# 0xPARC/plonkathon

Measured on NVIDIA H100. Metric: plonk_proofs_per_s_2^20_gates, higher is better.
Workload: dtype u256 (BN254 Fr/Fq integers, 8x32-bit Montgomery limbs)

## Files before the change

### plonkathon_b200/csrc/curve.cuh

```cuda
#pragma once
#include "field.cuh"

namespace pb200 {

struct alignas(16) G1Affine {
  Fq x, y;
};

struct alignas(16) G1XYZZ {
  Fq X, Y, ZZ, ZZZ;
  PB_HD bool is_inf() const { return ZZ.is_zero(); }
  static PB_HD G1XYZZ identity() {
    G1XYZZ r;
    r.X = Fq::zero(); r.Y = Fq::zero(); r.ZZ = Fq::zero(); r.ZZZ = Fq::zero();
    return r;
  }
};

PB_HD G1XYZZ g1_from_affine(const G1Affine& p) {
  G1XYZZ r;
  r.X = p.x; r.Y = p.y; r.ZZ = Fq::one(); r.ZZZ = Fq::one();
  return r;
}

PB_HD void g1_double_affine(G1XYZZ& acc, const G1Affine& p) {
  Fq U = fp_dbl(p.y);
  Fq V = fp_sqr(U);
  Fq W = fp_mul(U, V);
  Fq S = fp_mul(p.x, V);
  Fq M = fp_sqr(p.x);
  M = fp_add(fp_dbl(M), M);
  Fq X3 = fp_sub(fp_sqr(M), fp_dbl(S));
  acc.Y = fp_sub(fp_mul(M, fp_sub(S, X3)), fp_mul(W, p.y));
  acc.X = X3;
  acc.ZZ = V;
  acc.ZZZ = W;
}

PB_HD void g1_double(G1XYZZ& a) {
  if (a.is_inf()) return;
  Fq U = fp_dbl(a.Y);
  Fq V = fp_sqr(U);
  Fq W = fp_mul(U, V);
  Fq S = fp_mul(a.X, V);
  Fq M = fp_sqr(a.X);
  M = fp_add(fp_dbl(M), M);
  Fq X3 = fp_sub(fp_sqr(M), fp_dbl(S));
  a.Y = fp_sub(fp_mul(M, fp_sub(S, X3)), fp_mul(W, a.Y));
  a.X = X3;
  a.ZZ = fp_mul(V, a.ZZ);
  a.ZZZ = fp_mul(W, a.ZZZ);
}

PB_HD void g1_add_mixed(G1XYZZ& acc, const G1Affine& p) {
  if (acc.is_inf()) {
    acc = g1_from_affine(p);
    return;
  }
  Fq U2 = fp_mul(p.x, acc.ZZ);
  Fq S2 = fp_mul(p.y, acc.ZZZ);
  Fq Pd = fp_sub(U2, acc.X);
  Fq Rd = fp_sub(S2, acc.Y);
  if (Pd.is_zero()) {
    if (Rd.is_zero()) g1_double_affine(acc, p);
    else acc = G1XYZZ::identity();
    return;
  }
  Fq PP = fp_sqr(Pd);
  Fq PPP = fp_mul(Pd, PP);
  Fq Q = fp_mul(acc.X, PP);
  Fq X3 = fp_sub(fp_sub(fp_sqr(Rd), PPP), fp_dbl(Q));
  acc.Y = fp_sub(fp_mul(Rd, fp_sub(Q, X3)), fp_mul(acc.Y, PPP));
  acc.X = X3;
  acc.ZZ = fp_mul(acc.ZZ, PP);
  acc.ZZZ = fp_mul(acc.ZZZ, PPP);
}

PB_HD void g1_add_mixed_uniform(G1XYZZ& acc, const G1Affine& p) {
  const bool was_inf = acc.is_inf();
  Fq U2 = fp_mul(p.x, acc.ZZ);
  Fq S2 = fp_mul(p.y, acc.ZZZ);
  Fq Pd = fp_sub(U2, acc.X);
  Fq Rd = fp_sub(S2, acc.Y);
  if (!was_inf && Pd.is_zero()) {
    if (Rd.is_zero()) g1_double_affine(acc, p);
    else acc = G1XYZZ::identity();
    return;
  }
  Fq PP = fp_sqr(Pd);
  Fq PPP = fp_mul(Pd, PP);
  Fq Q = fp_mul(acc.X, PP);
  Fq X3 = fp_sub(fp_sub(fp_sqr(Rd), PPP), fp_dbl(Q));
  Fq Y3 = fp_sub(fp_mul(Rd, fp_sub(Q, X3)), fp_mul(acc.Y, PPP));
  Fq ZZ3 = fp_mul(acc.ZZ, PP);
  Fq ZZZ3 = fp_mul(acc.ZZZ, PPP);
  const Fq one = Fq::one();
#pragma unroll
  for (int i = 0; i < 8; i++) {
    acc.X.v[i] = was_inf ? p.x.v[i] : X3.v[i];
    acc.Y.v[i] = was_inf ? p.y.v[i] : Y3.v[i];
    acc.ZZ.v[i] = was_inf ? one.v[i] : ZZ3.v[i];
    acc.ZZZ.v[i] = was_inf ? one.v[i] : ZZZ3.v[i];
  }
}

PB_HD void g1_add(G1XYZZ& acc, const G1XYZZ& q) {
  if (q.is_inf()) return;
  if (acc.is_inf()) {
    acc = q;
    return;
  }
  Fq U1 = fp_mul(acc.X, q.ZZ);
  Fq U2 = fp_mul(q.X, acc.ZZ);
  Fq S1 = fp_mul(acc.Y, q.ZZZ);
  Fq S2 = fp_mul(q.Y, acc.ZZZ);
  Fq Pd = fp_sub(U2, U1);
  Fq Rd = fp_sub(S2, S1);
  if (Pd.is_zero()) {
    if (Rd.is_zero()) g1_double(acc);
    else acc = G1XYZZ::identity();
    return;
  }
  Fq PP = fp_sqr(Pd);
  Fq PPP = fp_mul(Pd, PP);
  Fq Q = fp_mul(U1, PP);
  Fq X3 = fp_sub(fp_sub(fp_sqr(Rd), PPP), fp_dbl(Q));
  acc.Y = fp_sub(fp_mul(Rd, fp_sub(Q, X3)), fp_mul(S1, PPP));
  acc.X = X3;
  acc.ZZ = fp_mul(fp_mul(acc.ZZ, q.ZZ), PP);
  acc.ZZZ = fp_mul(fp_mul(acc.ZZZ, q.ZZZ), PPP);
}

PB_HD void g1_add_uniform(G1XYZZ& acc, const G1XYZZ& q) {
  const bool a_inf = acc.is_inf(), q_inf = q.is_inf();
  Fq U1 = fp_mul(acc.X, q.ZZ);
  Fq U2 = fp_mul(q.X, acc.ZZ);
  Fq S1 = fp_mul(acc.Y, q.ZZZ);
  Fq S2 = fp_mul(q.Y, acc.ZZZ);
  Fq Pd = fp_sub(U2, U1);
  Fq Rd = fp_sub(S2, S1);
  if (!a_inf && !q_inf && Pd.is_zero()) {
    if (Rd.is_zero()) g1_double(acc);
    else acc = G1XYZZ::identity();
    return;
  }
  Fq PP = fp_sqr(Pd);
  Fq PPP = fp_mul(Pd, PP);
  Fq Q = fp_mul(U1, PP);
  Fq X3 = fp_sub(fp_sub(fp_sqr(Rd), PPP), fp_dbl(Q));
  Fq Y3 = fp_sub(fp_mul(Rd, fp_sub(Q, X3)), fp_mul(S1, PPP));
  Fq ZZ3 = fp_mul(fp_mul(acc.ZZ, q.ZZ), PP);
  Fq ZZZ3 = fp_mul(fp_mul(acc.ZZZ, q.ZZZ), PPP);
#pragma unroll
  for (int i = 0; i < 8; i++) {
    acc.X.v[i] = q_inf ? acc.X.v[i] : (a_inf ? q.X.v[i] : X3.v[i]);
    acc.Y.v[i] = q_inf ? acc.Y.v[i] : (a_inf ? q.Y.v[i] : Y3.v[i]);
    acc.ZZ.v[i] = q_inf ? acc.ZZ.v[i] : (a_inf ? q.ZZ.v[i] : ZZ3.v[i]);
    acc.ZZZ.v[i] = q_inf ? acc.ZZZ.v[i] : (a_inf ? q.ZZZ.v[i] : ZZZ3.v[i]);
  }
}

PB_HD G1Affine g1_neg_affine(const G1Affine& p) {
  G1Affine r;
  r.x = p.x;
  r.y = fp_neg(p.y);
  return r;
}

PB_HD bool g1_to_affine(const G1XYZZ& a, G1Affine& out) {
  if (a.is_inf()) {
    out.x = Fq::zero();
    out.y = Fq::zero();
    return true;
  }
  Fq A = fp_inv(a.ZZZ);
  Fq izz = fp_sqr(fp_mul(a.ZZ, A));
  out.x = fp_mul(a.X, izz);
  out.y = fp_mul(a.Y, A);
  return false;
}

}
```

### plonkathon_b200/csrc/field.cuh

```cuda
#pragma once
#include <stdint.h>

#if defined(__CUDACC__)
#define PB_HD __host__ __device__ __forceinline__
#define PB_D __device__ __forceinline__
#else
#define PB_HD inline
#define PB_D inline
#endif

namespace pb200 {

#if defined(__CUDA_ARCH__)
PB_D uint32_t add_cc(uint32_t a, uint32_t b) { uint32_t r; asm volatile("add.cc.u32 %0, %1, %2;" : "=r"(r) : "r"(a), "r"(b)); return r; }
PB_D uint32_t addc_cc(uint32_t a, uint32_t b) { uint32_t r; asm volatile("addc.cc.u32 %0, %1, %2;" : "=r"(r) : "r"(a), "r"(b)); return r; }
PB_D uint32_t addc(uint32_t a, uint32_t b) { uint32_t r; asm volatile("addc.u32 %0, %1, %2;" : "=r"(r) : "r"(a), "r"(b)); return r; }
PB_D uint32_t sub_cc(uint32_t a, uint32_t b) { uint32_t r; asm volatile("sub.cc.u32 %0, %1, %2;" : "=r"(r) : "r"(a), "r"(b)); return r; }
PB_D uint32_t subc_cc(uint32_t a, uint32_t b) { uint32_t r; asm volatile("subc.cc.u32 %0, %1, %2;" : "=r"(r) : "r"(a), "r"(b)); return r; }
PB_D uint32_t subc(uint32_t a, uint32_t b) { uint32_t r; asm volatile("subc.u32 %0, %1, %2;" : "=r"(r) : "r"(a), "r"(b)); return r; }
PB_D uint32_t mul_lo(uint32_t a, uint32_t b) { uint32_t r; asm volatile("mul.lo.u32 %0, %1, %2;" : "=r"(r) : "r"(a), "r"(b)); return r; }
PB_D uint32_t mul_hi(uint32_t a, uint32_t b) { uint32_t r; asm volatile("mul.hi.u32 %0, %1, %2;" : "=r"(r) : "r"(a), "r"(b)); return r; }
PB_D uint32_t mad_lo_cc(uint32_t a, uint32_t b, uint32_t c) { uint32_t r; asm volatile("mad.lo.cc.u32 %0, %1, %2, %3;" : "=r"(r) : "r"(a), "r"(b), "r"(c)); return r; }
PB_D uint32_t madc_lo_cc(uint32_t a, uint32_t b, uint32_t c) { uint32_t r; asm volatile("madc.lo.cc.u32 %0, %1, %2, %3;" : "=r"(r) : "r"(a), "r"(b), "r"(c)); return r; }
PB_D uint32_t madc_hi_cc(uint32_t a, uint32_t b, uint32_t c) { uint32_t r; asm volatile("madc.hi.cc.u32 %0, %1, %2, %3;" : "=r"(r) : "r"(a), "r"(b), "r"(c)); return r; }
// ... 143 lines not shown
      U[j] = madc_lo_cc(a[j], b, U[j]);
      U[j + 1] = madc_hi_cc(a[j], b, U[j + 1]);
    }
    uint32_t c1 = addc(0u, 0u);
    w = V[1];
    V[0] = mad_lo_cc(a[1], b, V[2]);
    V[1] = madc_hi_cc(a[1], b, V[3]);
    V[2] = madc_lo_cc(a[3], b, V[4]);
    V[3] = madc_hi_cc(a[3], b, V[5]);
    V[4] = madc_lo_cc(a[5], b, V[6]);
    V[5] = madc_hi_cc(a[5], b, V[7]);
    V[6] = madc_lo_cc(a[7], b, 0u);
    V[7] = madc_hi(a[7], b, c1);
  }
  uint32_t m = mul_lo(U[0] + w, P::NP0);
  fp_mad_row_mod<P, 1>(V, m);
  fp_mad_row_mod<P, 0>(U, m);
  V[7] = addc(V[7], 0u);
}

#if !defined(__CUDA_ARCH__) && defined(PB_HOST_FAST_MUL)
template <class P>
inline Fp<P> fp_mul_host64(const Fp<P>& a, const Fp<P>& b) {
  typedef unsigned __int128 u128;
  uint64_t A[4], B[4], M[4], T[6] = {0, 0, 0, 0, 0, 0};
  for (int i = 0; i < 4; i++) {
    A[i] = (uint64_t)a.v[2 * i] | ((uint64_t)a.v[2 * i + 1] << 32);
    B[i] = (uint64_t)b.v[2 * i] | ((uint64_t)b.v[2 * i + 1] << 32);
    M[i] = (uint64_t)P::p(2 * i) | ((uint64_t)P::p(2 * i + 1) << 32);
  }
  uint64_t np = 1;
  for (int k = 0; k < 6; k++) np *= 2 - M[0] * np;
  np = (uint64_t)0 - np;
  for (int i = 0; i < 4; i++) {
    u128 c = 0;
    for (int j = 0; j < 4; j++) { c += (u128)A[j] * B[i] + T[j]; T[j] = (uint64_t)c; c >>= 64; }
    c += T[4]; T[4] = (uint64_t)c; T[5] = (uint64_t)(c >> 64);
    uint64_t m = T[0] * np;
    c = (u128)m * M[0] + T[0]; c >>= 64;
    for (int j = 1; j < 4; j++) { c += (u128)m * M[j] + T[j]; T[j - 1] = (uint64_t)c; c >>= 64; }
    c += T[4]; T[3] = (uint64_t)c; T[4] = T[5] + (uint64_t)(c >> 64); T[5] = 0;
  }
  uint64_t r[4]; u128 br = 0; bool ge = T[4] != 0;
  if (!ge) { ge = true; for (int i = 3; i >= 0; i--) { if (T[i] != M[i]) { ge = T[i] > M[i]; break; } } }
  if (ge) { for (int i = 0; i < 4; i++) { u128 d = (u128)T[i] - M[i] - (uint64_t)br; r[i] = (uint64_t)d; br = (d >> 64) & 1; } }
  else { for (int i = 0; i < 4; i++) r[i] = T[i]; }
  Fp<P> o;
  for (int i = 0; i < 4; i++) { o.v[2 * i] = (uint32_t)r[i]; o.v[2 * i + 1] = (uint32_t)(r[i] >> 32); }
  return o;
}
#endif

template <class P>
PB_HD Fp<P> fp_mul(const Fp<P>& a, const Fp<P>& b) {
#if !defined(__CUDA_ARCH__) && defined(PB_HOST_FAST_MUL)
  return fp_mul_host64(a, b);
#else
  uint32_t X[8], Y[8], w;
  fp_cios_step<P, true>(X, Y, w, a.v, b.v[0]);
  fp_cios_step<P, false>(Y, X, w, a.v, b.v[1]);
  fp_cios_step<P, false>(X, Y, w, a.v, b.v[2]);
  fp_cios_step<P, false>(Y, X, w, a.v, b.v[3]);
  fp_cios_step<P, false>(X, Y, w, a.v, b.v[4]);
  fp_cios_step<P, false>(Y, X, w, a.v, b.v[5]);
  fp_cios_step<P, false>(X, Y, w, a.v, b.v[6]);
  fp_cios_step<P, false>(Y, X, w, a.v, b.v[7]);
  Fp<P> r;
  (void)add_cc(w, 0xffffffffu);
  r.v[0] = addc_cc(X[0], Y[1]);
#pragma unroll
  for (int i = 1; i < 7; i++) r.v[i] = addc_cc(X[i], Y[i + 1]);
  r.v[7] = addc(X[7], 0u);
  fp_reduce_once(r);
  return r;
#endif
}

template <class P>
PB_HD Fp<P> fp_sqr(const Fp<P>& a) { return fp_mul(a, a); }

template <class P>
PB_HD Fp<P> fp_to_mont(const Fp<P>& a) { return fp_mul(a, Fp<P>::r2()); }

template <class P>
PB_HD Fp<P> fp_to_mont_any(const Fp<P>& a) { return fp_mul(Fp<P>::r2(), a); }

template <class P>
PB_HD Fp<P> fp_from_mont(const Fp<P>& a) {
  Fp<P> o = Fp<P>::zero();
  o.v[0] = 1;
  return fp_mul(a, o);
}

template <class P>
PB_HD Fp<P> fp_pow(const Fp<P>& a, const uint32_t* e) {
  Fp<P> r = Fp<P>::one();
  bool started = false;
  for (int i = 255; i >= 0; i--) {
    if (started) r = fp_sqr(r);
    if ((e[i >> 5] >> (i & 31)) & 1) {
      r = started ? fp_mul(r, a) : a;
      started = true;
    }
  }
  return r;
}

template <class P>
PB_HD Fp<P> fp_pow_u64(const Fp<P>& a, uint64_t e) {
  uint32_t ee[8] = {(uint32_t)e, (uint32_t)(e >> 32), 0, 0, 0, 0, 0, 0};
  return fp_pow(a, ee);
}

template <class P>
PB_HD Fp<P> fp_inv(const Fp<P>& a) {
  uint32_t e[8];
#pragma unroll
  for (int i = 0; i < 8; i++) e[i] = P::p(i);
  e[0] -= 2;
  return fp_pow(a, e);
}

typedef Fp<FrParams> Fr;
typedef Fp<FqParams> Fq;

}
```

### plonkathon_b200/csrc/host_selftest.cpp

```cpp
#include "field.cuh"
#include "curve.cuh"
#include "msm_digits.cuh"
#include "modinv.cuh"
#include "msm_bucket.cuh"
#include "msm_sort.cuh"
#include "ntt_shard.cuh"
#include <algorithm>
#include <vector>
#include <cstring>
using namespace pb200;

template <class F> static F ld(const uint32_t* p) { F r; memcpy(r.v, p, 32); return r; }
template <class F> static void st(uint32_t* p, const F& a) { memcpy(p, a.v, 32); }

extern "C" {
int hs_field_op(int field, int op, const uint32_t* a, const uint32_t* b, uint32_t* out) {
#define RUN(F)                                                   \
  {                                                              \
    F x = ld<F>(a), y = ld<F>(b), r;                             \
    switch (op) {                                                \
      case 0: r = fp_add(x, y); break;                           \
      case 1: r = fp_sub(x, y); break;                           \
      case 2: r = fp_mul(x, y); break;                           \
      case 3: r = fp_neg(x); break;                              \
      case 4: r = fp_inv(x); break;                              \
      case 5: r = fp_to_mont(x); break;                          \
      case 6: r = fp_from_mont(x); break;                        \
      case 7: r = fp_dbl(x); break;                              \
      case 8: r = fp_sqr(x); break;                              \
      case 9: r = fp_inv_gcd(x); break;                          \
      case 10: r = fp_inv_plain_gcd(x); break;                   \
      default: return -1;                                        \
    }                                                            \
    st(out, r);                                                  \
  }
  if (field == 0) RUN(Fr) else RUN(Fq)
  return 0;
}

int hs_small_dft(int log_g, const uint32_t* x, const uint32_t* tw, uint32_t* out) {
  DftTw t;
  for (int k = 0; k < 4; k++) t.w[k] = ld<Fr>(tw + 8 * k);
#define RUN_DFT(LG)                                                     \
  {                                                                     \
    Fr v[1 << LG];                                                      \
    for (int i = 0; i < (1 << LG); i++) v[i] = ld<Fr>(x + 8 * i);       \
    small_dft<LG>(v, t);                                                \
    for (int i = 0; i < (1 << LG); i++) st(out + 8 * i, v[i]);          \
  }
  switch (log_g) {
    case 1: RUN_DFT(1) break;
    case 2: RUN_DFT(2) break;
    case 3: RUN_DFT(3) break;
    default: return -1;
  }
#undef RUN_DFT
  return 0;
}

int hs_msm_digits(const uint32_t* scalar, uint32_t c, int32_t* digits, uint32_t* n_windows) {
  MsmGeom g;
  g.c = c;
  g.W = (256 + c - 1) / c;
  g.half = 1u << (c - 1);
  g.fixed_base = 0;
  g.point_stride = 0;
  g.batch = 1;
  g.lo = 0;
  g.nloc = g.half;
  g.own_log = 0;
  g.own_rank = 0;
  g.sets = g.W;
  g.nb = g.half * g.W;
  Fr s = ld<Fr>(scalar);
  DigitWalk dw(&s, 0, 0);
  for (uint32_t w = 0; w < g.W; w++) {
    uint32_t neg, d = dw.next(w, g, neg);
    digits[w] = neg ? -(int32_t)d : (int32_t)d;
  }
  *n_windows = g.W;
  return (int)dw.carry;
}

int hs_curve_op(int op, const uint32_t* acc_in, const uint32_t* other, int other_inf, uint32_t* out) {
  G1XYZZ acc;
  memcpy(&acc, acc_in, sizeof(acc));
  switch (op) {
    case 0: {
      G1Affine p;
// ... 314 lines not shown
```

### plonkathon_b200/csrc/msm.cu

```cuda
#include <algorithm>
#include <cstring>

#include "common.cuh"
#include "comm.cuh"
#include "msm_bucket.cuh"
#include "msm_digits.cuh"
#include "msm_sort.cuh"

namespace pb200 {

__device__ __forceinline__ G1Affine ld_affine(const G1Affine* p) {
  const uint4* q = reinterpret_cast<const uint4*>(p);
  uint4 a = __ldg(q), b = __ldg(q + 1), c = __ldg(q + 2), d = __ldg(q + 3);
  G1Affine r;
  r.x.v[0] = a.x; r.x.v[1] = a.y; r.x.v[2] = a.z; r.x.v[3] = a.w;
  r.x.v[4] = b.x; r.x.v[5] = b.y; r.x.v[6] = b.z; r.x.v[7] = b.w;
  r.y.v[0] = c.x; r.y.v[1] = c.y; r.y.v[2] = c.z; r.y.v[3] = c.w;
  r.y.v[4] = d.x; r.y.v[5] = d.y; r.y.v[6] = d.z; r.y.v[7] = d.w;
  return r;
}

__device__ __forceinline__ uint32_t block_exclusive_scan(uint32_t v, uint32_t* sh, uint32_t* total) {
  const uint32_t lane = threadIdx.x & 31, wid = threadIdx.x >> 5, nw = blockDim.x >> 5;
  uint32_t x = v;
// ... 124 lines not shown
  __shared__ uint32_t sh[8];
  uint32_t base = blockIdx.x * PB_SCAN_TILE + threadIdx.x * 8;
  uint32_t c[8];
  uint32_t s = 0;
  for (int k = 0; k < 8; k++) { c[k] = base + k < nb ? (counts[base + k] + pad) & ~pad : 0; s += c[k]; }
  uint32_t total;
  uint32_t run = tile_sums[blockIdx.x] + block_exclusive_scan(s, sh, &total);
  for (int k = 0; k < 8; k++) {
    if (base + k < nb) { offsets[base + k] = run; counts[base + k] = 0; }
    run += c[k];
  }
}

__global__ void __launch_bounds__(256) k_msm_chunk_map(SortArgs a) {
  __shared__ uint32_t sh[8];
  uint32_t total;
  const uint32_t run = block_exclusive_scan(chunk_map_sum(a, threadIdx.x), sh, &total);
  chunk_map_write(a, threadIdx.x, run, total);
}

__global__ void __launch_bounds__(128, 4) k_aff_round0(AffAcc a) {
  Fq pref[PB_AFF_BMAX];
  uint32_t desc[PB_AFF_BMAX];
  aff_round0_thread(a, (uint64_t)blockIdx.x * blockDim.x + threadIdx.x, pref, desc);
}
__global__ void __launch_bounds__(128, 4) k_aff_round(AffAcc a) {
  Fq pref[PB_AFF_BMAX];
  uint32_t desc[PB_AFF_BMAX];
  aff_round_thread(a, (uint64_t)blockIdx.x * blockDim.x + threadIdx.x, pref, desc);
}
__global__ void __launch_bounds__(256) k_aff_tail(AffAcc a, uint64_t s_bound) {
  Fq pref[PB_AFF_BMAX];
  uint32_t desc[PB_AFF_BMAX];
  const uint32_t maxc = *a.max_cnt;
  for (uint32_t r = PB_AFF_GRID_ROUNDS; r < 32 && maxc > (1u << r); r++) {
    a.r = r;
    const uint64_t T = aff_round_threads(s_bound, a.B, r);
    for (uint64_t t = threadIdx.x; t < T; t += blockDim.x) aff_round_thread(a, t, pref, desc);
    __syncthreads();
  }
}

#define PB_MSM_EMPTY 0xffffffffu

__device__ __forceinline__ uint32_t upper_bound_u32(const uint32_t* a, uint32_t n, uint32_t key) {
  uint32_t lo = 0, hi = n;
  while (lo < hi) {
    uint32_t mid = (lo + hi) >> 1;
    if (__ldg(a + mid) > key) hi = mid; else lo = mid + 1;
  }
  return lo;
}

__global__ void __launch_bounds__(128) k_msm_seg_accumulate(const G1Affine* points, const uint32_t* offsets,
                                                            const uint32_t* sorted, uint32_t nb, uint32_t L,
                                                            G1XYZZ* buckets, G1XYZZ* slots, uint32_t* slot_bucket,
                                                            uint32_t* own_slot) {
  const uint32_t t = blockIdx.x * blockDim.x + threadIdx.x;
  const uint32_t M = offsets[nb];
  const uint64_t s64 = (uint64_t)t * L;
  if (s64 >= M) return;
  const uint32_t s = (uint32_t)s64;
  const uint32_t e = (uint32_t)min((uint64_t)M, s64 + L);
  uint32_t b = upper_bound_u32(offsets, nb + 1, s) - 1;
  uint32_t bstart = offsets[b], bend = offsets[b + 1];
  bool first = true;
  G1XYZZ acc = G1XYZZ::identity();
  for (uint32_t pos = s; pos <= e; pos++) {
    if (pos == bend || pos == e) {
      if (bstart >= s && bend <= e) {
        buckets[b] = acc;
      } else {
        uint32_t slot = first ? 2 * t : 2 * t + 1;
        slots[slot] = acc;
        slot_bucket[slot] = b;
        if (bstart >= s) own_slot[t] = slot;
      }
      if (pos == e) break;
      first = false;
      acc = G1XYZZ::identity();
      b++;
      while (offsets[b + 1] <= pos) b++;
      bstart = offsets[b];
      bend = offsets[b + 1];
    }
    uint32_t v = __ldg(sorted + pos);
    G1Affine p = ld_affine(points + (v & 0x7fffffffu));
    if (v >> 31) p.y = fp_neg(p.y);
    g1_add_mixed_uniform(acc, p);
  }
}

struct HeavyItem { uint32_t bucket, own_slot, t0, t1, piece_base, pieces; };
struct HeavyPiece { uint32_t item, index; };
#define PB_STITCH_PIECE 1024

__global__ void __launch_bounds__(128) k_msm_stitch(const uint32_t* offsets, uint32_t nb, uint32_t L,
                                                    uint32_t n_segments, const G1XYZZ* slots,
                                                    const uint32_t* slot_bucket, const uint32_t* own_slot,
                                                    G1XYZZ* buckets, HeavyItem* heavy, uint32_t* heavy_count,
                                                    HeavyPiece* pieces, uint32_t small_limit) {
  const uint32_t t = blockIdx.x * blockDim.x + threadIdx.x;
  if (t >= n_segments) return;
  const uint32_t os = own_slot[t];
  if (os == PB_MSM_EMPTY) return;
  const uint32_t b = slot_bucket[os];
  const uint32_t t1 = (offsets[b + 1] - 1) / L;
// ... 727 lines not shown
```

### plonkathon_b200/csrc/msm_bucket.cuh

```cuda
#pragma once
#include "curve.cuh"
#include "modinv.cuh"
#if !defined(__CUDA_ARCH__)
#include <stdio.h>
#include <stdlib.h>
#endif

namespace pb200 {

#define PB_AFF_ADD 1u
#define PB_AFF_DBL 2u
#define PB_AFF_INDEX_BITS 29
#define PB_AFF_INDEX_MASK ((1u << PB_AFF_INDEX_BITS) - 1)
#define PB_AFF_BMAX 128
#define PB_MSM_PAD 0xffffffffu
#define PB_AFF_GRID_ROUNDS 12

struct AffAcc {
  const G1Affine* table;
  const uint32_t* sorted;
  G1Affine* pts;
  const uint32_t* off;
  const uint32_t* cnt;
  const uint32_t* max_cnt;
// ... 152 lines not shown
    const uint32_t m0 = (aff_ld_u32(a.cnt + b) + 1) >> 1;
    if (m0 <= hs) continue;
    uint64_t u = lo > base ? (((uint64_t)(lo - base) + step - 1) >> r) << r : 0;
    for (; base + u < hi && u + hs < m0; u += step) {
      const uint32_t left = base + (uint32_t)u, right = left + (uint32_t)hs;
      const Fq x1 = aff_ld_fq_rw(&a.pts[left].x), x2 = aff_ld_fq_rw(&a.pts[right].x);
      if (aff_is_identity_x(x2)) continue;
      if (aff_is_identity_x(x1)) {
        G1Affine q;
        q.x = x2;
        q.y = aff_ld_fq_rw(&a.pts[right].y);
        aff_st_point(a.pts + left, q);
        continue;
      }
      Fq d = fp_sub(x2, x1);
      uint32_t kind = PB_AFF_ADD;
      if (d.is_zero()) {
        kind = aff_classify_equal_x(aff_ld_fq_rw(&a.pts[left].y), aff_ld_fq_rw(&a.pts[right].y), d);
        if (kind == 0) {
          aff_st_point(a.pts + left, aff_identity());
          continue;
        }
      }
#if !defined(__CUDA_ARCH__)
      if (K >= a.B) { fprintf(stderr, "aff_round_thread: chain longer than B\n"); abort(); }
#endif
      pref[K] = acc;
      desc[K] = left | (kind << PB_AFF_INDEX_BITS);
      K++;
      acc = fp_mul(acc, d);
    }
  }
  Fq inv = fp_inv_gcd(acc);
  while (K > 0) {
    K--;
    const uint32_t left = desc[K] & PB_AFF_INDEX_MASK, kind = desc[K] >> PB_AFF_INDEX_BITS;
    const uint32_t right = left + (uint32_t)hs;
    G1Affine p, q;
    p.x = aff_ld_fq_rw(&a.pts[left].x); p.y = aff_ld_fq_rw(&a.pts[left].y);
    q.x = aff_ld_fq_rw(&a.pts[right].x); q.y = aff_ld_fq_rw(&a.pts[right].y);
    const Fq d = kind == PB_AFF_ADD ? fp_sub(q.x, p.x) : fp_dbl(p.y);
    const Fq dinv = fp_mul(inv, pref[K]);
    inv = fp_mul(inv, d);
    aff_st_point(a.pts + left, aff_finish(p, q, kind, dinv));
  }
}

struct SR {
  G1XYZZ S, R;
};

PB_HD void g1_add_mixed_sel(G1XYZZ& acc, const G1Affine& p, bool take) {
  const bool was_inf = acc.is_inf();
  Fq U2 = fp_mul(p.x, acc.ZZ);
  Fq S2 = fp_mul(p.y, acc.ZZZ);
  Fq Pd = fp_sub(U2, acc.X);
  Fq Rd = fp_sub(S2, acc.Y);
  if (take && !was_inf && Pd.is_zero()) {
    if (Rd.is_zero()) g1_double_affine(acc, p);
    else acc = G1XYZZ::identity();
    return;
  }
  Fq PP = fp_sqr(Pd);
  Fq PPP = fp_mul(Pd, PP);
  Fq Q = fp_mul(acc.X, PP);
  Fq X3 = fp_sub(fp_sub(fp_sqr(Rd), PPP), fp_dbl(Q));
  Fq Y3 = fp_sub(fp_mul(Rd, fp_sub(Q, X3)), fp_mul(acc.Y, PPP));
  Fq ZZ3 = fp_mul(acc.ZZ, PP);
  Fq ZZZ3 = fp_mul(acc.ZZZ, PPP);
  const Fq one = Fq::one();
#pragma unroll
  for (int i = 0; i < 8; i++) {
    acc.X.v[i] = !take ? acc.X.v[i] : (was_inf ? p.x.v[i] : X3.v[i]);
    acc.Y.v[i] = !take ? acc.Y.v[i] : (was_inf ? p.y.v[i] : Y3.v[i]);
    acc.ZZ.v[i] = !take ? acc.ZZ.v[i] : (was_inf ? one.v[i] : ZZ3.v[i]);
    acc.ZZZ.v[i] = !take ? acc.ZZZ.v[i] : (was_inf ? one.v[i] : ZZZ3.v[i]);
  }
}

struct ReduceArgs {
  const G1Affine* pts;
  const uint32_t* off;
  const uint32_t* cnt;
  const G1XYZZ* xb;
  SR* out;
  uint32_t sets;
  uint32_t m;
  uint32_t g;
};
PB_HD uint32_t reduce_groups(uint32_t m, uint32_t g) { return (m + g - 1) / g; }

PB_HD void reduce_level0_fetch(const ReduceArgs& a, uint32_t b, G1XYZZ& acc) {
  if (a.xb) {
    const G1XYZZ v = a.xb[b];
    g1_add_uniform(acc, v);
    return;
  }
  const bool live = aff_ld_u32(a.cnt + b) != 0;
  const uint32_t slot = live ? aff_ld_u32(a.off + b) >> 1 : 0;
  G1Affine p;
  p.x = aff_ld_fq(&a.pts[slot].x);
  p.y = aff_ld_fq(&a.pts[slot].y);
  g1_add_mixed_sel(acc, p, live && !aff_is_identity_x(p.x));
}

PB_HD void reduce_level0_thread(const ReduceArgs& a, uint64_t t) {
  const uint32_t groups = reduce_groups(a.m, a.g);
  if (t >= (uint64_t)a.sets * groups) return;
  const uint32_t set = (uint32_t)(t / groups), gi = (uint32_t)(t % groups);
  const uint32_t j0 = gi * a.g;
  const uint32_t len = a.m - j0 < a.g ? a.m - j0 : a.g;
  const uint32_t b0 = set * a.m + j0;
  G1XYZZ acc = G1XYZZ::identity(), sum = G1XYZZ::identity();
  reduce_level0_fetch(a, b0 + len - 1, acc);
  for (uint32_t k = len; k-- > 0;) {
    G1XYZZ nxt = acc;
    if (k > 0) reduce_level0_fetch(a, b0 + k - 1, nxt);
    g1_add_uniform(sum, acc);
    acc = nxt;
  }
  SR o;
  o.S = acc;
  o.R = sum;
  a.out[t] = o;
}

#if defined(__CUDA_ARCH__)
static __device__ __noinline__ void blk_add(G1XYZZ& acc, const G1XYZZ& q) { g1_add(acc, q); }
static __device__ __noinline__ void blk_double(G1XYZZ& a) { g1_double(a); }
// ... 76 lines not shown
```

Before: 20.83.

## Use lazy Montgomery reduction, fused dual-product mul and dedicated squaring in EC adds

Adds lazy (unreduced, below 2p) Montgomery multiply, subtract, negate and zero-test variants, a fused a*b+c*d CIOS multiply, and a dedicated squaring that computes the wide product before reduction. The XYZZ add and double formulas are rewritten around a shared tail that uses these, skipping many final conditional subtractions. It also sets a min-blocks launch bound on the segment-accumulate kernel. The lazy paths depend on BN254's headroom under 2^256, and the launch bound may force register spills.

```diff
diff --git a/plonkathon_b200/csrc/curve.cuh b/plonkathon_b200/csrc/curve.cuh
--- a/plonkathon_b200/csrc/curve.cuh
+++ b/plonkathon_b200/csrc/curve.cuh
@@ -31,7 +31,8 @@
   Fq M = fp_sqr(p.x);
   M = fp_add(fp_dbl(M), M);
   Fq X3 = fp_sub(fp_sqr(M), fp_dbl(S));
-  acc.Y = fp_sub(fp_mul(M, fp_sub(S, X3)), fp_mul(W, p.y));
+  acc.Y = fp_mul2_lazy(M, fp_sub(S, X3), W, fp_neg_lazy(p.y));
+  fp_reduce_once(acc.Y);
   acc.X = X3;
   acc.ZZ = V;
   acc.ZZZ = W;
@@ -46,10 +47,23 @@
   Fq M = fp_sqr(a.X);
   M = fp_add(fp_dbl(M), M);
   Fq X3 = fp_sub(fp_sqr(M), fp_dbl(S));
-  a.Y = fp_sub(fp_mul(M, fp_sub(S, X3)), fp_mul(W, a.Y));
+  a.Y = fp_mul2_lazy(M, fp_sub(S, X3), W, fp_neg_lazy(a.Y));
+  fp_reduce_once(a.Y);
   a.X = X3;
   a.ZZ = fp_mul(V, a.ZZ);
   a.ZZZ = fp_mul(W, a.ZZZ);
+}
+
+PB_HD void g1_add_tail(const Fq& U1, const Fq& S1, const Fq& Pd, const Fq& Rd, const Fq& Z2, const Fq& Z3, G1XYZZ& r) {
+  const Fq PP = fp_sqr_lazy(Pd);
+  r.ZZ = fp_mul(Z2, PP);
+  const Fq PPP = fp_mul_lazy(Pd, PP);
+  r.ZZZ = fp_mul(Z3, PPP);
+  const Fq Q = fp_mul_lazy(U1, PP);
+  r.X = fp_sub_lazy(fp_sub_lazy(fp_sub_lazy(fp_sqr_lazy(Rd), PPP), Q), Q);
+  fp_reduce_once(r.X);
+  r.Y = fp_mul2_lazy(Rd, fp_sub(Q, r.X), fp_neg_lazy(S1), PPP);
+  fp_reduce_once(r.Y);
 }
 
 PB_HD void g1_add_mixed(G1XYZZ& acc, const G1Affine& p) {
@@ -57,50 +71,40 @@
     acc = g1_from_affine(p);
     return;
   }
-  Fq U2 = fp_mul(p.x, acc.ZZ);
-  Fq S2 = fp_mul(p.y, acc.ZZZ);
+  Fq U2 = fp_mul_lazy(p.x, acc.ZZ);
+  Fq S2 = fp_mul_lazy(p.y, acc.ZZZ);
   Fq Pd = fp_sub(U2, acc.X);
   Fq Rd = fp_sub(S2, acc.Y);
-  if (Pd.is_zero()) {
-    if (Rd.is_zero()) g1_double_affine(acc, p);
+  if (fp_is_zero_lazy(Pd)) {
+    if (fp_is_zero_lazy(Rd)) g1_double_affine(acc, p);
     else acc = G1XYZZ::identity();
     return;
   }
-  Fq PP = fp_sqr(Pd);
-  Fq PPP = fp_mul(Pd, PP);
-  Fq Q = fp_mul(acc.X, PP);
-  Fq X3 = fp_sub(fp_sub(fp_sqr(Rd), PPP), fp_dbl(Q));
-  acc.Y = fp_sub(fp_mul(Rd, fp_sub(Q, X3)), fp_mul(acc.Y, PPP));
-  acc.X = X3;
-  acc.ZZ = fp_mul(acc.ZZ, PP);
-  acc.ZZZ = fp_mul(acc.ZZZ, PPP);
+  G1XYZZ r;
+  g1_add_tail(acc.X, acc.Y, Pd, Rd, acc.ZZ, acc.ZZZ, r);
+  acc = r;
 }
 
 PB_HD void g1_add_mixed_uniform(G1XYZZ& acc, const G1Affine& p) {
   const bool was_inf = acc.is_inf();
-  Fq U2 = fp_mul(p.x, acc.ZZ);
-  Fq S2 = fp_mul(p.y, acc.ZZZ);
+  Fq U2 = fp_mul_lazy(p.x, acc.ZZ);
+  Fq S2 = fp_mul_lazy(p.y, acc.ZZZ);
   Fq Pd = fp_sub(U2, acc.X);
   Fq Rd = fp_sub(S2, acc.Y);
-  if (!was_inf && Pd.is_zero()) {
-    if (Rd.is_zero()) g1_double_affine(acc, p);
+  if (!was_inf && fp_is_zero_lazy(Pd)) {
+    if (fp_is_zero_lazy(Rd)) g1_double_affine(acc, p);
     else acc = G1XYZZ::identity();
     return;
   }
-  Fq PP = fp_sqr(Pd);
-  Fq PPP = fp_mul(Pd, PP);
-  Fq Q = fp_mul(acc.X, PP);
-  Fq X3 = fp_sub(fp_sub(fp_sqr(Rd), PPP), fp_dbl(Q));
-  Fq Y3 = fp_sub(fp_mul(Rd, fp_sub(Q, X3)), fp_mul(acc.Y, PPP));
-  Fq ZZ3 = fp_mul(acc.ZZ, PP);
-  Fq ZZZ3 = fp_mul(acc.ZZZ, PPP);
+  G1XYZZ r;
+  g1_add_tail(acc.X, acc.Y, Pd, Rd, acc.ZZ, acc.ZZZ, r);
   const Fq one = Fq::one();
 #pragma unroll
   for (int i = 0; i < 8; i++) {
-    acc.X.v[i] = was_inf ? p.x.v[i] : X3.v[i];
-    acc.Y.v[i] = was_inf ? p.y.v[i] : Y3.v[i];
-    acc.ZZ.v[i] = was_inf ? one.v[i] : ZZ3.v[i];
-    acc.ZZZ.v[i] = was_inf ? one.v[i] : ZZZ3.v[i];
+    acc.X.v[i] = was_inf ? p.x.v[i] : r.X.v[i];
+    acc.Y.v[i] = was_inf ? p.y.v[i] : r.Y.v[i];
+    acc.ZZ.v[i] = was_inf ? one.v[i] : r.ZZ.v[i];
+    acc.ZZZ.v[i] = was_inf ? one.v[i] : r.ZZZ.v[i];
   }
 }
 
@@ -111,52 +115,42 @@
     return;
   }
   Fq U1 = fp_mul(acc.X, q.ZZ);
-  Fq U2 = fp_mul(q.X, acc.ZZ);
+  Fq U2 = fp_mul_lazy(q.X, acc.ZZ);
   Fq S1 = fp_mul(acc.Y, q.ZZZ);
-  Fq S2 = fp_mul(q.Y, acc.ZZZ);
+  Fq S2 = fp_mul_lazy(q.Y, acc.ZZZ);
   Fq Pd = fp_sub(U2, U1);
   Fq Rd = fp_sub(S2, S1);
-  if (Pd.is_zero()) {
-    if (Rd.is_zero()) g1_double(acc);
+  if (fp_is_zero_lazy(Pd)) {
+    if (fp_is_zero_lazy(Rd)) g1_double(acc);
     else acc = G1XYZZ::identity();
     return;
   }
-  Fq PP = fp_sqr(Pd);
-  Fq PPP = fp_mul(Pd, PP);
-  Fq Q = fp_mul(U1, PP);
-  Fq X3 = fp_sub(fp_sub(fp_sqr(Rd), PPP), fp_dbl(Q));
-  acc.Y = fp_sub(fp_mul(Rd, fp_sub(Q, X3)), fp_mul(S1, PPP));
-  acc.X = X3;
-  acc.ZZ = fp_mul(fp_mul(acc.ZZ, q.ZZ), PP);
-  acc.ZZZ = fp_mul(fp_mul(acc.ZZZ, q.ZZZ), PPP);
+  G1XYZZ r;
+  g1_add_tail(U1, S1, Pd, Rd, fp_mul_lazy(acc.ZZ, q.ZZ), fp_mul_lazy(acc.ZZZ, q.ZZZ), r);
+  acc = r;
 }
 
 PB_HD void g1_add_uniform(G1XYZZ& acc, const G1XYZZ& q) {
   const bool a_inf = acc.is_inf(), q_inf = q.is_inf();
   Fq U1 = fp_mul(acc.X, q.ZZ);
-  Fq U2 = fp_mul(q.X, acc.ZZ);
+  Fq U2 = fp_mul_lazy(q.X, acc.ZZ);
   Fq S1 = fp_mul(acc.Y, q.ZZZ);
-  Fq S2 = fp_mul(q.Y, acc.ZZZ);
+  Fq S2 = fp_mul_lazy(q.Y, acc.ZZZ);
   Fq Pd = fp_sub(U2, U1);
   Fq Rd = fp_sub(S2, S1);
-  if (!a_inf && !q_inf && Pd.is_zero()) {
-    if (Rd.is_zero()) g1_double(acc);
+  if (!a_inf && !q_inf && fp_is_zero_lazy(Pd)) {
+    if (fp_is_zero_lazy(Rd)) g1_double(acc);
     else acc = G1XYZZ::identity();
     return;
   }
-  Fq PP = fp_sqr(Pd);
-  Fq PPP = fp_mul(Pd, PP);
-  Fq Q = fp_mul(U1, PP);
-  Fq X3 = fp_sub(fp_sub(fp_sqr(Rd), PPP), fp_dbl(Q));
-  Fq Y3 = fp_sub(fp_mul(Rd, fp_sub(Q, X3)), fp_mul(S1, PPP));
-  Fq ZZ3 = fp_mul(fp_mul(acc.ZZ, q.ZZ), PP);
-  Fq ZZZ3 = fp_mul(fp_mul(acc.ZZZ, q.ZZZ), PPP);
+  G1XYZZ r;
+  g1_add_tail(U1, S1, Pd, Rd, fp_mul_lazy(acc.ZZ, q.ZZ), fp_mul_lazy(acc.ZZZ, q.ZZZ), r);
 #pragma unroll
   for (int i = 0; i < 8; i++) {
-    acc.X.v[i] = q_inf ? acc.X.v[i] : (a_inf ? q.X.v[i] : X3.v[i]);
-    acc.Y.v[i] = q_inf ? acc.Y.v[i] : (a_inf ? q.Y.v[i] : Y3.v[i]);
-    acc.ZZ.v[i] = q_inf ? acc.ZZ.v[i] : (a_inf ? q.ZZ.v[i] : ZZ3.v[i]);
-    acc.ZZZ.v[i] = q_inf ? acc.ZZZ.v[i] : (a_inf ? q.ZZZ.v[i] : ZZZ3.v[i]);
+    acc.X.v[i] = q_inf ? acc.X.v[i] : (a_inf ? q.X.v[i] : r.X.v[i]);
+    acc.Y.v[i] = q_inf ? acc.Y.v[i] : (a_inf ? q.Y.v[i] : r.Y.v[i]);
+    acc.ZZ.v[i] = q_inf ? acc.ZZ.v[i] : (a_inf ? q.ZZ.v[i] : r.ZZ.v[i]);
+    acc.ZZZ.v[i] = q_inf ? acc.ZZZ.v[i] : (a_inf ? q.ZZZ.v[i] : r.ZZZ.v[i]);
   }
 }
 
diff --git a/plonkathon_b200/csrc/field.cuh b/plonkathon_b200/csrc/field.cuh
--- a/plonkathon_b200/csrc/field.cuh
+++ b/plonkathon_b200/csrc/field.cuh
@@ -219,6 +219,17 @@
 #endif
 
 template <class P>
+PB_HD Fp<P> fp_cios_final(const uint32_t* X, const uint32_t* Y, uint32_t w) {
+  Fp<P> r;
+  (void)add_cc(w, 0xffffffffu);
+  r.v[0] = addc_cc(X[0], Y[1]);
+#pragma unroll
+  for (int i = 1; i < 7; i++) r.v[i] = addc_cc(X[i], Y[i + 1]);
+  r.v[7] = addc(X[7], 0u);
+  return r;
+}
+
+template <class P>
 PB_HD Fp<P> fp_mul(const Fp<P>& a, const Fp<P>& b) {
 #if !defined(__CUDA_ARCH__) && defined(PB_HOST_FAST_MUL)
   return fp_mul_host64(a, b);
@@ -232,19 +243,239 @@
   fp_cios_step<P, false>(Y, X, w, a.v, b.v[5]);
   fp_cios_step<P, false>(X, Y, w, a.v, b.v[6]);
   fp_cios_step<P, false>(Y, X, w, a.v, b.v[7]);
+  Fp<P> r = fp_cios_final<P>(X, Y, w);
+  fp_reduce_once(r);
+  return r;
+#endif
+}
+
+template <class P>
+PB_HD Fp<P> fp_mul_lazy(const Fp<P>& a, const Fp<P>& b) {
+#if !defined(__CUDA_ARCH__) && defined(PB_HOST_FAST_MUL)
+  return fp_mul_host64(a, b);
+#else
+  uint32_t X[8], Y[8], w;
+  fp_cios_step<P, true>(X, Y, w, a.v, b.v[0]);
+  fp_cios_step<P, false>(Y, X, w, a.v, b.v[1]);
+  fp_cios_step<P, false>(X, Y, w, a.v, b.v[2]);
+  fp_cios_step<P, false>(Y, X, w, a.v, b.v[3]);
+  fp_cios_step<P, false>(X, Y, w, a.v, b.v[4]);
+  fp_cios_step<P, false>(Y, X, w, a.v, b.v[5]);
+  fp_cios_step<P, false>(X, Y, w, a.v, b.v[6]);
+  fp_cios_step<P, false>(Y, X, w, a.v, b.v[7]);
+  return fp_cios_final<P>(X, Y, w);
+#endif
+}
+
+template <class P>
+PB_HD constexpr uint32_t fp_2p(int i) { return (P::p(i) << 1) | (i ? P::p(i - 1) >> 31 : 0u); }
+
+template <class P>
+PB_HD Fp<P> fp_sub_lazy(const Fp<P>& a, const Fp<P>& b) {
   Fp<P> r;
-  (void)add_cc(w, 0xffffffffu);
-  r.v[0] = addc_cc(X[0], Y[1]);
-#pragma unroll
-  for (int i = 1; i < 7; i++) r.v[i] = addc_cc(X[i], Y[i + 1]);
-  r.v[7] = addc(X[7], 0u);
+  r.v[0] = sub_cc(a.v[0], b.v[0]);
+#pragma unroll
+  for (int i = 1; i < 8; i++) r.v[i] = subc_cc(a.v[i], b.v[i]);
+  uint32_t mask = subc(0u, 0u);
+  r.v[0] = add_cc(r.v[0], fp_2p<P>(0) & mask);
+#pragma unroll
+  for (int i = 1; i < 7; i++) r.v[i] = addc_cc(r.v[i], fp_2p<P>(i) & mask);
+  r.v[7] = addc(r.v[7], fp_2p<P>(7) & mask);
+  return r;
+}
+
+template <class P>
+PB_HD Fp<P> fp_neg_lazy(const Fp<P>& a) {
+  Fp<P> r;
+  r.v[0] = sub_cc(P::p(0), a.v[0]);
+#pragma unroll
+  for (int i = 1; i < 7; i++) r.v[i] = subc_cc(P::p(i), a.v[i]);
+  r.v[7] = subc(P::p(7), a.v[7]);
+  return r;
+}
+
+template <class P>
+PB_HD bool fp_is_zero_lazy(const Fp<P>& a) {
+  uint32_t z = 0, q = 0;
+#pragma unroll
+  for (int i = 0; i < 8; i++) { z |= a.v[i]; q |= a.v[i] ^ P::p(i); }
+  return z == 0 || q == 0;
+}
+
+template <class P, bool FIRST>
+PB_HD void fp_cios_step2(uint32_t* U, uint32_t* V, uint32_t& w, const uint32_t* a, uint32_t b, const uint32_t* c,
+                         uint32_t d) {
+  if (FIRST) {
+#pragma unroll
+    for (int j = 0; j < 8; j += 2) {
+      U[j] = mul_lo(a[j], b);
+      U[j + 1] = mul_hi(a[j], b);
+      V[j] = mul_lo(a[j + 1], b);
+      V[j + 1] = mul_hi(a[j + 1], b);
+    }
+    w = 0;
+  } else {
+    (void)add_cc(w, 0xffffffffu);
+    U[0] = madc_lo_cc(a[0], b, U[0]);
+    U[1] = madc_hi_cc(a[0], b, U[1]);
+#pragma unroll
+    for (int j = 2; j < 8; j += 2) {
+      U[j] = madc_lo_cc(a[j], b, U[j]);
+      U[j + 1] = madc_hi_cc(a[j], b, U[j + 1]);
+    }
+    uint32_t c1 = addc(0u, 0u);
+    w = V[1];
+    V[0] = mad_lo_cc(a[1], b, V[2]);
+    V[1] = madc_hi_cc(a[1], b, V[3]);
+    V[2] = madc_lo_cc(a[3], b, V[4]);
+    V[3] = madc_hi_cc(a[3], b, V[5]);
+    V[4] = madc_lo_cc(a[5], b, V[6]);
+    V[5] = madc_hi_cc(a[5], b, V[7]);
+    V[6] = madc_lo_cc(a[7], b, 0u);
+    V[7] = madc_hi(a[7], b, c1);
+  }
+  fp_mad_row<P>(V, c + 1, d);
+  fp_mad_row<P>(U, c, d);
+  V[7] = addc(V[7], 0u);
+  uint32_t m = mul_lo(U[0] + w, P::NP0);
+  fp_mad_row_mod<P, 1>(V, m);
+  fp_mad_row_mod<P, 0>(U, m);
+  V[7] = addc(V[7], 0u);
+}
+
+template <class P>
+PB_HD Fp<P> fp_mul2_lazy(const Fp<P>& a, const Fp<P>& b, const Fp<P>& c, const Fp<P>& d) {
+#if !defined(__CUDA_ARCH__) && defined(PB_HOST_FAST_MUL)
+  return fp_add(fp_mul_host64(a, b), fp_mul_host64(c, d));
+#else
+  uint32_t X[8], Y[8], w;
+  fp_cios_step2<P, true>(X, Y, w, a.v, b.v[0], c.v, d.v[0]);
+  fp_cios_step2<P, false>(Y, X, w, a.v, b.v[1], c.v, d.v[1]);
+  fp_cios_step2<P, false>(X, Y, w, a.v, b.v[2], c.v, d.v[2]);
+  fp_cios_step2<P, false>(Y, X, w, a.v, b.v[3], c.v, d.v[3]);
+  fp_cios_step2<P, false>(X, Y, w, a.v, b.v[4], c.v, d.v[4]);
+  fp_cios_step2<P, false>(Y, X, w, a.v, b.v[5], c.v, d.v[5]);
+  fp_cios_step2<P, false>(X, Y, w, a.v, b.v[6], c.v, d.v[6]);
+  fp_cios_step2<P, false>(Y, X, w, a.v, b.v[7], c.v, d.v[7]);
+  return fp_cios_final<P>(X, Y, w);
+#endif
+}
+
+
+PB_HD void fp_sqr_chain(uint32_t* acc, const uint32_t* x, uint32_t y, int n) {
+  acc[0] = mad_lo_cc(x[0], y, acc[0]);
+  acc[1] = madc_hi_cc(x[0], y, acc[1]);
+#pragma unroll
+  for (int k = 1; k < n; k++) {
+    acc[2 * k] = madc_lo_cc(x[2 * k], y, acc[2 * k]);
+    acc[2 * k + 1] = madc_hi_cc(x[2 * k], y, acc[2 * k + 1]);
+  }
+}
+
+PB_HD void fp_sqr_wide(uint32_t* T, const uint32_t* a) {
+  uint32_t E[16], O[16];
+#pragma unroll
+  for (int k = 0; k < 16; k++) { E[k] = 0; O[k] = 0; }
+  fp_sqr_chain(E + 2, a + 2, a[0], 3);
+  fp_sqr_chain(O + 0, a + 1, a[0], 4);
+  fp_sqr_chain(E + 4, a + 3, a[1], 3);
+  fp_sqr_chain(O + 2, a + 2, a[1], 3);
+  O[8] = addc(0u, 0u);
+  fp_sqr_chain(E + 6, a + 4, a[2], 2);
+  E[10] = addc(0u, 0u);
+  fp_sqr_chain(O + 4, a + 3, a[2], 3);
+  fp_sqr_chain(E + 8, a + 5, a[3], 2);
+  fp_sqr_chain(O + 6, a + 4, a[3], 2);
+  O[10] = addc(0u, 0u);
+  fp_sqr_chain(E + 10, a + 6, a[4], 1);
+  E[12] = addc(0u, 0u);
+  fp_sqr_chain(O + 8, a + 5, a[4], 2);
+  fp_sqr_chain(E + 12, a + 7, a[5], 1);
+  fp_sqr_chain(O + 10, a + 6, a[5], 1);
+  O[12] = addc(0u, 0u);
+  fp_sqr_chain(O + 12, a + 7, a[6], 1);
+  uint32_t S[16];
+  S[0] = 0;
+  S[1] = O[0];
+  S[2] = add_cc(E[2], O[1]);
+#pragma unroll
+  for (int k = 3; k < 14; k++) S[k] = addc_cc(E[k], O[k - 1]);
+  S[14] = addc_cc(O[13], 0u);
+  S[15] = addc(0u, 0u);
+  S[1] = add_cc(S[1], S[1]);
+#pragma unroll
+  for (int k = 2; k < 15; k++) S[k] = addc_cc(S[k], S[k]);
+  S[15] = addc(S[15], S[15]);
+  T[0] = mad_lo_cc(a[0], a[0], 0u);
+  T[1] = madc_hi_cc(a[0], a[0], S[1]);
+#pragma unroll
+  for (int i = 1; i < 7; i++) {
+    T[2 * i] = madc_lo_cc(a[i], a[i], S[2 * i]);
+    T[2 * i + 1] = madc_hi_cc(a[i], a[i], S[2 * i + 1]);
+  }
+  T[14] = madc_lo_cc(a[7], a[7], S[14]);
+  T[15] = madc_hi(a[7], a[7], S[15]);
+}
+
+template <class P, bool FIRST>
+PB_HD void fp_redc_step(uint32_t* U, uint32_t* V, uint32_t& w) {
+  uint32_t cf = 0;
+  if (FIRST) {
+#pragma unroll
+    for (int j = 0; j < 8; j++) V[j] = 0;
+    w = 0;
+  } else {
+    cf = w != 0;
+    w = V[1];
+#pragma unroll
+    for (int j = 0; j < 6; j++) V[j] = V[j + 2];
+    V[6] = 0;
+    V[7] = 0;
+  }
+  const uint32_t m = mul_lo(U[0] + w + cf, P::NP0);
+  fp_mad_row_mod<P, 1>(V, m);
+  (void)add_cc(cf, 0xffffffffu);
+  U[0] = madc_lo_cc(P::p(0), m, U[0]);
+  U[1] = madc_hi_cc(P::p(0), m, U[1]);
+#pragma unroll
+  for (int j = 2; j < 8; j += 2) {
+    U[j] = madc_lo_cc(P::p(j), m, U[j]);
+    U[j + 1] = madc_hi_cc(P::p(j), m, U[j + 1]);
+  }
+  V[7] = addc(V[7], 0u);
+}
+
+template <class P>
+PB_HD Fp<P> fp_sqr_lazy(const Fp<P>& a) {
+#if !defined(__CUDA_ARCH__) && defined(PB_HOST_FAST_MUL)
+  return fp_mul_host64(a, a);
+#else
+  uint32_t T[16], Y[8], w;
+  fp_sqr_wide(T, a.v);
+  uint32_t* X = T;
+  fp_redc_step<P, true>(X, Y, w);
+  fp_redc_step<P, false>(Y, X, w);
+  fp_redc_step<P, false>(X, Y, w);
+  fp_redc_step<P, false>(Y, X, w);
+  fp_redc_step<P, false>(X, Y, w);
+  fp_redc_step<P, false>(Y, X, w);
+  fp_redc_step<P, false>(X, Y, w);
+  fp_redc_step<P, false>(Y, X, w);
+  Fp<P> r = fp_cios_final<P>(X, Y, w);
+  r.v[0] = add_cc(r.v[0], T[8]);
+#pragma unroll
+  for (int i = 1; i < 7; i++) r.v[i] = addc_cc(r.v[i], T[8 + i]);
+  r.v[7] = addc(r.v[7], T[15]);
+  return r;
+#endif
+}
+
+template <class P>
+PB_HD Fp<P> fp_sqr(const Fp<P>& a) {
+  Fp<P> r = fp_sqr_lazy(a);
   fp_reduce_once(r);
   return r;
-#endif
-}
-
-template <class P>
-PB_HD Fp<P> fp_sqr(const Fp<P>& a) { return fp_mul(a, a); }
+}
 
 template <class P>
 PB_HD Fp<P> fp_to_mont(const Fp<P>& a) { return fp_mul(a, Fp<P>::r2()); }
diff --git a/plonkathon_b200/csrc/host_selftest.cpp b/plonkathon_b200/csrc/host_selftest.cpp
--- a/plonkathon_b200/csrc/host_selftest.cpp
+++ b/plonkathon_b200/csrc/host_selftest.cpp
@@ -30,11 +30,90 @@
       case 8: r = fp_sqr(x); break;                              \
       case 9: r = fp_inv_gcd(x); break;                          \
       case 10: r = fp_inv_plain_gcd(x); break;                   \
+      case 11: r = fp_mul_lazy(x, y); break;                     \
+      case 12: r = fp_sqr_lazy(x); break;                        \
+      case 13: r = fp_sub_lazy(x, y); break;                     \
+      case 14: r = fp_neg_lazy(x); break;                        \
+      case 15: r = fp_is_zero_lazy(x) ? F::one() : F::zero(); break; \
       default: return -1;                                        \
     }                                                            \
     st(out, r);                                                  \
   }
   if (field == 0) RUN(Fr) else RUN(Fq)
+#undef RUN
+  return 0;
+}
+
+int hs_field_mul2(int field, const uint32_t* a, const uint32_t* b, const uint32_t* c, const uint32_t* d, uint32_t* out) {
+  if (field == 0) st(out, fp_mul2_lazy(ld<Fr>(a), ld<Fr>(b), ld<Fr>(c), ld<Fr>(d)));
+  else st(out, fp_mul2_lazy(ld<Fq>(a), ld<Fq>(b), ld<Fq>(c), ld<Fq>(d)));
+  return 0;
+}
+}
+
+static Fq ref_sqr(const Fq& a) { return fp_mul(a, a); }
+static void ref_double(G1XYZZ& a) {
+  if (a.is_inf()) return;
+  Fq U = fp_dbl(a.Y), V = ref_sqr(U), W = fp_mul(U, V), S = fp_mul(a.X, V), M = ref_sqr(a.X);
+  M = fp_add(fp_dbl(M), M);
+  Fq X3 = fp_sub(ref_sqr(M), fp_dbl(S));
+  a.Y = fp_sub(fp_mul(M, fp_sub(S, X3)), fp_mul(W, a.Y));
+  a.X = X3;
+  a.ZZ = fp_mul(V, a.ZZ);
+  a.ZZZ = fp_mul(W, a.ZZZ);
+}
+static void ref_add_mixed(G1XYZZ& acc, const G1Affine& p) {
+  if (acc.is_inf()) { acc = g1_from_affine(p); return; }
+  Fq U2 = fp_mul(p.x, acc.ZZ), S2 = fp_mul(p.y, acc.ZZZ), Pd = fp_sub(U2, acc.X), Rd = fp_sub(S2, acc.Y);
+  if (Pd.is_zero()) {
+    if (Rd.is_zero()) { acc = g1_from_affine(p); ref_double(acc); }
+    else acc = G1XYZZ::identity();
+    return;
+  }
+  Fq PP = ref_sqr(Pd), PPP = fp_mul(Pd, PP), Q = fp_mul(acc.X, PP);
+  Fq X3 = fp_sub(fp_sub(ref_sqr(Rd), PPP), fp_dbl(Q));
+  acc.Y = fp_sub(fp_mul(Rd, fp_sub(Q, X3)), fp_mul(acc.Y, PPP));
+  acc.X = X3;
+  acc.ZZ = fp_mul(acc.ZZ, PP);
+  acc.ZZZ = fp_mul(acc.ZZZ, PPP);
+}
+static void ref_add(G1XYZZ& acc, const G1XYZZ& q) {
+  if (q.is_inf()) return;
+  if (acc.is_inf()) { acc = q; return; }
+  Fq U1 = fp_mul(acc.X, q.ZZ), U2 = fp_mul(q.X, acc.ZZ), S1 = fp_mul(acc.Y, q.ZZZ), S2 = fp_mul(q.Y, acc.ZZZ);
+  Fq Pd = fp_sub(U2, U1), Rd = fp_sub(S2, S1);
+  if (Pd.is_zero()) {
+    if (Rd.is_zero()) ref_double(acc);
+    else acc = G1XYZZ::identity();
+    return;
+  }
+  Fq PP = ref_sqr(Pd), PPP = fp_mul(Pd, PP), Q = fp_mul(U1, PP);
+  Fq X3 = fp_sub(fp_sub(ref_sqr(Rd), PPP), fp_dbl(Q));
+  acc.Y = fp_sub(fp_mul(Rd, fp_sub(Q, X3)), fp_mul(S1, PPP));
+  acc.X = X3;
+  acc.ZZ = fp_mul(fp_mul(acc.ZZ, q.ZZ), PP);
+  acc.ZZZ = fp_mul(fp_mul(acc.ZZZ, q.ZZZ), PPP);
+}
+
+extern "C" {
+int hs_curve_op_ref(int op, const uint32_t* acc_in, const uint32_t* other, int other_inf, uint32_t* out) {
+  G1XYZZ acc;
+  memcpy(&acc, acc_in, sizeof(acc));
+  if (op == 0 || op == 4) {
+    G1Affine p;
+    memcpy(&p.x, other, 32);
+    memcpy(&p.y, other + 8, 32);
+    if (!other_inf) ref_add_mixed(acc, p);
+  } else if (op == 1 || op == 5) {
+    G1XYZZ q;
+    memcpy(&q, other, sizeof(q));
+    ref_add(acc, q);
+  } else if (op == 2) {
+    ref_double(acc);
+  } else {
+    return -1;
+  }
+  memcpy(out, &acc, sizeof(acc));
   return 0;
 }
 
diff --git a/plonkathon_b200/csrc/msm.cu b/plonkathon_b200/csrc/msm.cu
--- a/plonkathon_b200/csrc/msm.cu
+++ b/plonkathon_b200/csrc/msm.cu
@@ -200,7 +200,7 @@
   return lo;
 }
 
-__global__ void __launch_bounds__(128) k_msm_seg_accumulate(const G1Affine* points, const uint32_t* offsets,
+__global__ void __launch_bounds__(128, 4) k_msm_seg_accumulate(const G1Affine* points, const uint32_t* offsets,
                                                             const uint32_t* sorted, uint32_t nb, uint32_t L,
                                                             G1XYZZ* buckets, G1XYZZ* slots, uint32_t* slot_bucket,
                                                             uint32_t* own_slot) {
diff --git a/plonkathon_b200/csrc/msm_bucket.cuh b/plonkathon_b200/csrc/msm_bucket.cuh
--- a/plonkathon_b200/csrc/msm_bucket.cuh
+++ b/plonkathon_b200/csrc/msm_bucket.cuh
@@ -228,29 +228,24 @@
 
 PB_HD void g1_add_mixed_sel(G1XYZZ& acc, const G1Affine& p, bool take) {
   const bool was_inf = acc.is_inf();
-  Fq U2 = fp_mul(p.x, acc.ZZ);
-  Fq S2 = fp_mul(p.y, acc.ZZZ);
+  Fq U2 = fp_mul_lazy(p.x, acc.ZZ);
+  Fq S2 = fp_mul_lazy(p.y, acc.ZZZ);
   Fq Pd = fp_sub(U2, acc.X);
   Fq Rd = fp_sub(S2, acc.Y);
-  if (take && !was_inf && Pd.is_zero()) {
-    if (Rd.is_zero()) g1_double_affine(acc, p);
+  if (take && !was_inf && fp_is_zero_lazy(Pd)) {
+    if (fp_is_zero_lazy(Rd)) g1_double_affine(acc, p);
     else acc = G1XYZZ::identity();
     return;
   }
-  Fq PP = fp_sqr(Pd);
-  Fq PPP = fp_mul(Pd, PP);
-  Fq Q = fp_mul(acc.X, PP);
-  Fq X3 = fp_sub(fp_sub(fp_sqr(Rd), PPP), fp_dbl(Q));
-  Fq Y3 = fp_sub(fp_mul(Rd, fp_sub(Q, X3)), fp_mul(acc.Y, PPP));
-  Fq ZZ3 = fp_mul(acc.ZZ, PP);
-  Fq ZZZ3 = fp_mul(acc.ZZZ, PPP);
+  G1XYZZ r;
+  g1_add_tail(acc.X, acc.Y, Pd, Rd, acc.ZZ, acc.ZZZ, r);
   const Fq one = Fq::one();
 #pragma unroll
   for (int i = 0; i < 8; i++) {
-    acc.X.v[i] = !take ? acc.X.v[i] : (was_inf ? p.x.v[i] : X3.v[i]);
-    acc.Y.v[i] = !take ? acc.Y.v[i] : (was_inf ? p.y.v[i] : Y3.v[i]);
-    acc.ZZ.v[i] = !take ? acc.ZZ.v[i] : (was_inf ? one.v[i] : ZZ3.v[i]);
-    acc.ZZZ.v[i] = !take ? acc.ZZZ.v[i] : (was_inf ? one.v[i] : ZZZ3.v[i]);
+    acc.X.v[i] = !take ? acc.X.v[i] : (was_inf ? p.x.v[i] : r.X.v[i]);
+    acc.Y.v[i] = !take ? acc.Y.v[i] : (was_inf ? p.y.v[i] : r.Y.v[i]);
+    acc.ZZ.v[i] = !take ? acc.ZZ.v[i] : (was_inf ? one.v[i] : r.ZZ.v[i]);
+    acc.ZZZ.v[i] = !take ? acc.ZZZ.v[i] : (was_inf ? one.v[i] : r.ZZZ.v[i]);
   }
 }
 
```

New measurement: 21.80, median of 6. 1.05x the previous value.
